# chansoopark98/Deep-Visual-SLAM

Measured on AMD Instinct MI355X. Metric: VO training-step frames/sec (3-frame 640x480 snippets), higher is better.
Workload: dtype f32; 1 GPU; configs[2]/[3]: full 4-scale photometric+smoothness loss, batch 12 per GPU, ResNet-18; per_gpu_batch=12, global_batch=12, num_scales=4, image=640x480, parallelism=dp1, streams=depth | pose | 2x weight-gradient, optimizer=fused Adam pass at lr 0: every step computes from the seeded weights, gpu_max_hw_queues=4

## Files before the change

### deep-visual-slam_amd/csrc/conv_common.h

```cpp
#pragma once
#include "common.h"

namespace dvsconv {

using f32x4 = __attribute__((ext_vector_type(4))) float;
using f32x16 = __attribute__((ext_vector_type(16))) float;

constexpr int BK = 32;
constexpr int LDK = BK + 4;
constexpr int NT = 256;

enum Act { ACT_NONE = 0, ACT_RELU = 1, ACT_ELU = 2, ACT_SIGMOID = 3, ACT_GELU = 4 };
enum Pad { PAD_ZERO = 0, PAD_REFLECT = 1 };
enum InMode {
    IN_NHWC = 0,
    IN_UPCAT = 1,
    IN_PLANAR = 2,
    IN_DGRAD = 3
};

struct ConvShape {
    int B, H, W, Cin;
    int Ho, Wo, Cout;
    int kh, kw, stride, pad;
// ... 161 lines not shown
    return v;
}

__device__ __forceinline__ f32x4 load_dy4(const float* __restrict__ dy, const ConvShape& s, const InXform& t, int b,
                                          int ty, int tx, int co) {
    size_t o = (((size_t)b * s.H + ty) * s.W + tx) * s.Cin + co;
    f32x4 v = *reinterpret_cast<const f32x4*>(dy + o);
    if (t.dact) {
        f32x4 y = *reinterpret_cast<const f32x4*>(t.aux + o);
#pragma unroll
        for (int j = 0; j < 4; ++j) v[j] *= act_grad_from_out(y[j], t.dact);
    }
    return v;
}

__device__ __forceinline__ f32x4 gather_dgrad_raw(const float* __restrict__ dy, const ConvShape& s, const InXform& t,
                                                  int b, int yp, int xp, int ky, int kx, int co, bool& ok, f32x4& yv,
                                                  f32x4& extra) {
    int ty = yp - ky, tx = xp - kx;
    if (s.stride == 2) {
        ok = ok && ((ty | tx) & 1) == 0;
        ty >>= 1;
        tx >>= 1;
    }
    const bool in_y = (unsigned)ty < (unsigned)s.H, in_x = (unsigned)tx < (unsigned)s.W;
    const bool row_ok = ok;
    ok = ok && in_y && in_x;
    size_t o = (((size_t)b * s.H + clampi(ty, s.H)) * s.W + clampi(tx, s.W)) * s.Cin + co;
    f32x4 v = *reinterpret_cast<const f32x4*>(dy + o);
    if (t.dact) yv = *reinterpret_cast<const f32x4*>(t.aux + o);
    extra = f32x4{0.f, 0.f, 0.f, 0.f};
    if (s.pad_mode == PAD_REFLECT) {
        int y = yp - 1, x = xp - 1;
        int ey = (y == 1 && ky == 0) ? 0 : ((y == s.H - 2 && ky == s.kh - 1) ? s.H - 1 : -1);
        int ex = (x == 1 && kx == 0) ? 0 : ((x == s.W - 2 && kx == s.kw - 1) ? s.W - 1 : -1);
        if (row_ok && (ey >= 0 || ex >= 0)) {
            if (ey >= 0 && in_x) extra += load_dy4(dy, s, t, b, ey, tx, co);
            if (ex >= 0 && in_y) extra += load_dy4(dy, s, t, b, ty, ex, co);
            if (ey >= 0 && ex >= 0) extra += load_dy4(dy, s, t, b, ey, ex, co);
        }
    }
    return v;
}

__device__ __forceinline__ f32x4 finalize_dgrad(f32x4 v, const f32x4& yv, const f32x4& extra, bool ok, int dact) {
#pragma unroll
    for (int j = 0; j < 4; ++j) {
        float u = dact ? v[j] * act_grad_from_out(yv[j], dact) : v[j];
        v[j] = (ok ? u : 0.f) + extra[j];
    }
    return v;
}

__device__ __forceinline__ f32x4 gather_planar_raw(const float* __restrict__ x, const ConvShape& s, int b, int iy0,
                                                   int ix0, int k, bool ok, unsigned& mask4, int& ci_out) {
    int kx = k & 7, row = k >> 3;
    int ci = row / s.kh, ky = row - ci * s.kh;
    ci = min(ci, s.Cin - 1);
    ci_out = ci;
    int iy = iy0 + ky;
    bool oky = ok && (unsigned)iy < (unsigned)s.H;
    const float* rowp = x + (((size_t)b * s.Cin + ci) * s.H + clampi(iy, s.H)) * s.W;
    f32x4 v;
    mask4 = 0;
#pragma unroll
    for (int e = 0; e < 4; ++e) {
        int ix = ix0 + kx + e;
        v[e] = rowp[clampi(ix, s.W)];
        mask4 |= (oky && (unsigned)ix < (unsigned)s.W && kx + e < s.kw) ? (1u << e) : 0u;
    }
    return v;
}

template <bool FOLD>
__device__ __forceinline__ f32x4 finalize_planar(f32x4 v, unsigned mask4, float sc, float sh) {
#pragma unroll
    for (int e = 0; e < 4; ++e) {
        float u = FOLD ? v[e] * sc + sh : v[e];
        v[e] = ((mask4 >> e) & 1u) ? u : 0.f;
    }
    return v;
}

template <int TM, int TN>
__device__ __forceinline__ void mfma_stage(const float* __restrict__ As, const float* __restrict__ Bs, int a_row0,
                                           int b_row0, int lane, f32x16 (&acc)[TM][TN]) {
    const int r = lane & 31, h = lane >> 5;
#pragma unroll
    for (int j = 0; j < BK / 8; ++j) {
        f32x4 a[TM], b[TN];
#pragma unroll
        for (int m = 0; m < TM; ++m)
            a[m] = *reinterpret_cast<const f32x4*>(As + (a_row0 + m * 32 + r) * LDK + j * 8 + h * 4);
#pragma unroll
        for (int n = 0; n < TN; ++n)
            b[n] = *reinterpret_cast<const f32x4*>(Bs + (b_row0 + n * 32 + r) * LDK + j * 8 + h * 4);
#pragma unroll
        for (int t = 0; t < 4; ++t)
#pragma unroll
            for (int m = 0; m < TM; ++m)
#pragma unroll
                for (int n = 0; n < TN; ++n)
                    acc[m][n] = __builtin_amdgcn_mfma_f32_32x32x2f32(a[m][t], b[n][t], acc[m][n], 0, 0, 0);
    }
}

using bf16x8 = __attribute__((ext_vector_type(8))) __bf16;
using bf16x4 = __attribute__((ext_vector_type(4))) __bf16;
constexpr int LDKH = BK + 8;
__device__ __forceinline__ bf16x4 to_bf16(f32x4 v) {
    return bf16x4{(__bf16)v[0], (__bf16)v[1], (__bf16)v[2], (__bf16)v[3]};
}
template <int TM, int TN>
__device__ __forceinline__ void mfma_stage_bf16(const __bf16* __restrict__ As, const __bf16* __restrict__ Bs, int a_row0, int b_row0,
                                                int lane, f32x16 (&acc)[TM][TN]) {
    const int r = lane & 31, h = lane >> 5;
#pragma unroll
    for (int j = 0; j < BK / 16; ++j) {
        bf16x8 a[TM], b[TN];
#pragma unroll
        for (int m = 0; m < TM; ++m) a[m] = *reinterpret_cast<const bf16x8*>(As + (a_row0 + m * 32 + r) * LDKH + j * 16 + h * 8);
#pragma unroll
        for (int n = 0; n < TN; ++n) b[n] = *reinterpret_cast<const bf16x8*>(Bs + (b_row0 + n * 32 + r) * LDKH + j * 16 + h * 8);
#pragma unroll
        for (int m = 0; m < TM; ++m)
#pragma unroll
            for (int n = 0; n < TN; ++n) acc[m][n] = __builtin_amdgcn_mfma_f32_32x32x16_bf16(a[m], b[n], acc[m][n], 0, 0, 0);
    }
}

constexpr int OOB_OFF = 0x7ffffff0;
__device__ __forceinline__ __amdgpu_buffer_rsrc_t dma_rsrc(const float* base, size_t bytes) {
    return __builtin_amdgcn_make_buffer_rsrc(const_cast<float*>(base), 0, (int)bytes, 0x00020000);
}
__device__ __forceinline__ void dma16_buf(__amdgpu_buffer_rsrc_t r, int voff_bytes, int soff_bytes, float* lds_wave_base) {
    __builtin_amdgcn_raw_ptr_buffer_load_lds(r, (__attribute__((address_space(3))) void*)lds_wave_base, 16, voff_bytes,
                                             soff_bytes, 0, 0);
}

bool stem_shape(const ConvShape& s);
void stem_wgrad(const float* x, const float* dy, float* dw, const ConvShape& s, const float* sc, const float* sh,
                hipStream_t st);
void stem_fwd(const float* x, const float* w, float* y, float* stats, int stat_groups, const ConvShape& s,
              const float* sc, const float* sh, hipStream_t st);

bool thin_wgrad_shape(const ConvShape& s, const InXform& t);
bool thin_wgrad(const float* x, const float* dy, float* dw, float* dbias, const ConvShape& s, const InXform& t,
                hipStream_t st);
bool thin_fwd(const float* x, const float* w, const float* bias, float* y, const ConvShape& s, const InXform& t, int act,
              hipStream_t st);
bool thin_dgrad(const float* dy, const float* wt, float* dx, const float* y_out, int dact, int B, int H, int W, int Cin,
                int Cout, int split_c1, float* dx_skip, hipStream_t st);

}
```

### deep-visual-slam_amd/csrc/conv_fwd.hip

```cpp
#include "conv_common.h"

#include <cstdlib>
#include <type_traits>

namespace {
using namespace dvsconv;

struct FwdParams {
    const float* x;
    const float* w;
    const float* bias;
    float* y;
    float* stats;
    int stat_split;
    float* y2;
    int split_c1;
    int dbg_nobarrier;
    const float* zero_page;
    const float* res;
    int stat_mask, stat_stride;
    int work_m;
    int ksplit;
    Grid3 g;
    ConvShape s;
// ... 578 lines not shown
    if (W == 3 && x == 1) v += at(y + 1, W + 1) + ((ey >= 0) ? at(ey, W + 1) : f32x4{0.f, 0.f, 0.f, 0.f});
    if (H == 3 && W == 3 && y == 1 && x == 1) v += at(H + 1, W + 1);
    return v;
}
__global__ __launch_bounds__(256) void reflect_fold_kernel(const float* __restrict__ G, float* __restrict__ dx,
                                                           float* __restrict__ dx_skip, int B, int H, int W, int C, int C1) {
    const int cv = C / 4;
    const size_t i = (size_t)blockIdx.x * 256 + threadIdx.x;
    if (C1 == 0) {
        if (i >= (size_t)B * H * W * cv) return;
        const int c = (int)(i % cv) * 4;
        size_t m = i / cv;
        const int x = (int)(m % W);
        m /= W;
        const int y = (int)(m % H), b = (int)(m / H);
        *reinterpret_cast<f32x4*>(dx + (((size_t)b * H + y) * W + x) * C + c) = folded_at(G, b, y, x, c, H, W, C);
        return;
    }
    const int H2 = H >> 1, W2 = W >> 1;
    if (i >= (size_t)B * H2 * W2 * cv) return;
    const int c = (int)(i % cv) * 4;
    size_t m = i / cv;
    const int x2 = (int)(m % W2);
    m /= W2;
    const int y2 = (int)(m % H2), b = (int)(m / H2);
    f32x4 v[4];
#pragma unroll
    for (int q = 0; q < 4; ++q) v[q] = folded_at(G, b, 2 * y2 + (q >> 1), 2 * x2 + (q & 1), c, H, W, C);
    if (c < C1) {
        *reinterpret_cast<f32x4*>(dx + (((size_t)b * H2 + y2) * W2 + x2) * C1 + c) = (v[0] + v[1]) + (v[2] + v[3]);
    } else {
        const int cs = C - C1;
#pragma unroll
        for (int q = 0; q < 4; ++q)
            *reinterpret_cast<f32x4*>(dx_skip + (((size_t)b * H + 2 * y2 + (q >> 1)) * W + 2 * x2 + (q & 1)) * cs + (c - C1)) = v[q];
    }
}

struct PackEntry {
    const float* w;
    float* wt;
    int Cout, Cin, T, wg_begin;
};
__global__ __launch_bounds__(256) void pack_wt_batch_kernel(const PackEntry* __restrict__ tab, int n) {
    __shared__ float tile[32][33];
    __shared__ int s_e;
    if (threadIdx.x == 0) {
        int e = 0;
        while (e + 1 < n && (int)blockIdx.x >= tab[e + 1].wg_begin) ++e;
        s_e = e;
    }
    __syncthreads();
    const PackEntry en = tab[s_e];
    const int tci = (en.Cin + 31) / 32, tco = (en.Cout + 31) / 32;
    int local = blockIdx.x - en.wg_begin;
    const int tap = local / (tci * tco);
    local -= tap * tci * tco;
    const int co0 = (local / tci) * 32, ci0 = (local % tci) * 32;
    const int tx = threadIdx.x & 31, ty = threadIdx.x >> 5;
#pragma unroll
    for (int j = 0; j < 4; ++j) {
        int co = co0 + ty + 8 * j, ci = ci0 + tx;
        tile[ty + 8 * j][tx] = (co < en.Cout && ci < en.Cin) ? en.w[((size_t)co * en.T + tap) * en.Cin + ci] : 0.f;
    }
    __syncthreads();
#pragma unroll
    for (int j = 0; j < 4; ++j) {
        int ci = ci0 + ty + 8 * j, co = co0 + tx;
        if (ci < en.Cin && co < en.Cout) en.wt[((size_t)ci * en.T + tap) * en.Cout + co] = tile[tx][ty + 8 * j];
    }
}

}

extern "C" {

int dvs_reflect_fold(const float* g_padded, float* dx, float* dx_skip, int B, int H, int W, int C, int C1, void* stream) {
    DVS_REQUIRE(g_padded && dx && B > 0 && H >= 3 && W >= 3 && C > 0 && (C & 3) == 0, "dvs_reflect_fold: bad argument");
    DVS_REQUIRE(C1 == 0 || ((C1 & 3) == 0 && C1 <= C && !((H | W) & 1) && (C1 == C || dx_skip)), "dvs_reflect_fold: bad split");
    const size_t n = (C1 == 0 ? (size_t)B * H * W : (size_t)B * (H / 2) * (W / 2)) * (C / 4);
    hipStream_t st = static_cast<hipStream_t>(stream);
    dvs::ProfScope prof(dvs::SLOT_CONV_DGRAD, st);
    hipLaunchKernelGGL(reflect_fold_kernel, dim3((unsigned)((n + 255) / 256)), dim3(256), 0, st, g_padded, dx, dx_skip, B, H, W, C, C1);
    return dvs::check_launch("dvs_reflect_fold");
}

int dvs_act_bwd(const float* dy, const float* y, float* dz, size_t n, int act, float* dbias, int C, void* stream) {
    DVS_REQUIRE(dy && y && dz && n > 0 && (n & 3) == 0 && act >= 0 && act <= 3, "dvs_act_bwd: bad argument");
    DVS_REQUIRE(!dbias || (C >= 4 && (C & 3) == 0 && C / 4 <= 256 && 256 % (C / 4) == 0 && n % C == 0),
                "dvs_act_bwd: the bias gradient needs C/4 to divide 256 (C=%d)", C);
    const size_t nvec = n / 4;
    size_t blocks = (nvec + 255) / 256;
    if (blocks > 512) blocks = 512;
    if (dbias) {
        size_t few = nvec / (256 * 32);
        few = few < 32 ? 32 : few;
        if (blocks > few) blocks = few;
    }
    hipStream_t st = static_cast<hipStream_t>(stream);
    dvs::ProfScope prof(dvs::SLOT_CONV_DGRAD, st);
    hipLaunchKernelGGL(act_bwd_kernel, dim3((unsigned)blocks), dim3(256), 0, st, dy, y, dz, nvec, act, dbias, C);
    return dvs::check_launch("dvs_act_bwd");
}

int dvs_conv2d_pack_wt_batch(const void* table, int n_entries, int total_workgroups, void* stream) {
    DVS_REQUIRE(table && n_entries > 0 && total_workgroups > 0, "dvs_conv2d_pack_wt_batch: bad argument");
    hipLaunchKernelGGL(pack_wt_batch_kernel, dim3(total_workgroups), dim3(256), 0, static_cast<hipStream_t>(stream),
                       static_cast<const PackEntry*>(table), n_entries);
    return dvs::check_launch("dvs_conv2d_pack_wt_batch");
}

int dvs_conv2d_pack_wt(const float* w, float* wt, int Cout, int Cin, int kh, int kw, void* stream) {
    DVS_REQUIRE(w && wt && Cout > 0 && Cin > 0 && kh > 0 && kw > 0, "dvs_conv2d_pack_wt: bad argument");
    dim3 grid((Cin + 31) / 32, (Cout + 31) / 32, kh * kw);
    hipLaunchKernelGGL(pack_wt_kernel, grid, dim3(256), 0, static_cast<hipStream_t>(stream), w, wt, Cout, Cin, kh * kw);
    return dvs::check_launch("dvs_conv2d_pack_wt");
}

int dvs_conv2d_dgrad(const float* dy, const float* wt, float* dx, const dvs_conv_desc* d, const float* y_out,
                     int dact, float* dx_skip, int C1, const float* residual, void* stream) {
    DVS_REQUIRE(dy && wt && dx && d, "dvs_conv2d_dgrad: null pointer");
    DVS_REQUIRE(!residual || (C1 == 0 && residual != dx), "dvs_conv2d_dgrad: a residual excludes the upsample+concat split and may not alias dx");
    DVS_REQUIRE(C1 == 0 || (d->stride == 1 && (d->H & 1) == 0 && (d->W & 1) == 0 && C1 <= d->Cin &&
                            (C1 == d->Cin || dx_skip != nullptr)),
                "dvs_conv2d_dgrad: bad upsample+concat split");
    DVS_REQUIRE(d->stride == 1 || d->stride == 2, "dvs_conv2d_dgrad: stride %d (1 or 2 supported)", d->stride);
    DVS_REQUIRE((d->Cout & 3) == 0 && (d->Cin & 3) == 0, "dvs_conv2d_dgrad: channel counts must be multiples of 4");
    DVS_REQUIRE(d->pad_mode == PAD_ZERO || (d->pad_mode == 2 && d->pad == 0 && d->stride == 1 && d->H > 2 && d->W > 2 && !dact && !C1) ||
                    (d->pad_mode == PAD_REFLECT && d->pad == 1 && d->kh == 3 && d->kw == 3 && d->stride == 1 && d->H >= 2 && d->W >= 2),
                "dvs_conv2d_dgrad: reflect mode is ReflectionPad2d(1) + 3x3 stride 1 only; pad_mode 2 = pre-padded input, pad 0");
    DVS_REQUIRE(!dact || y_out, "dvs_conv2d_dgrad: activation gradient needs the forward output");
    DVS_REQUIRE((double)d->B * d->H * d->W * (d->Cin > d->Cout ? d->Cin : d->Cout) < 2147483648.0,
                "dvs_conv2d_dgrad: tensors must have fewer than 2^31 elements (32-bit gather offsets)");
    FwdParams p{};
    p.x = dy; p.w = wt; p.y = dx;
    p.stat_split = 0x7fffffff;
    ConvShape& s = p.s;
    int Ho = (d->H + 2 * d->pad - d->kh) / d->stride + 1, Wo = (d->W + 2 * d->pad - d->kw) / d->stride + 1;
    s.B = d->B;
    s.Ho = d->H; s.Wo = d->W; s.Cout = d->Cin;
    s.H = Ho; s.W = Wo; s.Cin = d->Cout;
    s.kh = d->kh; s.kw = d->kw; s.stride = d->stride; s.pad = d->pad; s.pad_mode = d->pad_mode;
    if (d->pad_mode == 2) {
        s.pad_mode = PAD_ZERO;
        p.work_m = d->B * (d->H - 2) * (d->W - 2);
    }
    s.Ktot = d->kh * d->kw * d->Cout;
    p.t.aux = y_out;
    p.t.dact = dact;
    p.y2 = dx_skip;
    p.split_c1 = C1;
    p.res = residual;
    hipStream_t st = static_cast<hipStream_t>(stream);
    if (!residual && d->pad_mode == PAD_REFLECT && d->kh == 3 && d->kw == 3 && d->stride == 1 && d->pad == 1 &&
        thin_dgrad(dy, wt, dx, y_out, dact, d->B, d->H, d->W, d->Cin, d->Cout, C1, dx_skip, st))
        return dvs::check_launch("dvs_conv2d_dgrad");
    launch_mode<IN_DGRAD, false>(p, st, dvs::SLOT_CONV_DGRAD);
    return dvs::check_launch("dvs_conv2d_dgrad");
}

int dvs_conv2d_fwd(const float* x, const float* w, const float* bias, float* y, const dvs_conv_desc* d,
                   const dvs_conv_fusion* f, void* stream) {
    DVS_REQUIRE(x && w && y && d, "dvs_conv2d_fwd: null pointer");
    DVS_REQUIRE(d->B > 0 && d->H > 0 && d->W > 0 && d->Cin > 0 && d->Cout > 0 && d->kh > 0 && d->kw > 0 &&
                    d->stride > 0 && d->pad >= 0,
                "dvs_conv2d_fwd: bad descriptor");
    FwdParams p{};
    p.x = x; p.w = w; p.bias = bias; p.y = y;
    p.stat_split = 0x7fffffff;
    ConvShape& s = p.s;
    s.B = d->B; s.H = d->H; s.W = d->W; s.Cin = d->Cin; s.Cout = d->Cout;
    s.kh = d->kh; s.kw = d->kw; s.stride = d->stride; s.pad = d->pad; s.pad_mode = d->pad_mode;
    s.Ho = (d->H + 2 * d->pad - d->kh) / d->stride + 1;
    s.Wo = (d->W + 2 * d->pad - d->kw) / d->stride + 1;
    DVS_REQUIRE(s.Ho > 0 && s.Wo > 0, "dvs_conv2d_fwd: empty output");
    DVS_REQUIRE((double)d->B * d->H * d->W * d->Cin < 2147483648.0 && (double)d->B * s.Ho * s.Wo * d->Cout < 2147483648.0,
                "dvs_conv2d_fwd: tensors must have fewer than 2^31 elements (32-bit gather offsets)");
    DVS_REQUIRE(d->pad_mode == PAD_ZERO || (d->pad < d->H && d->pad < d->W), "dvs_conv2d_fwd: reflect pad too large");
    int planar = 0;
    if (f) {
        p.t.x2 = f->x2; p.t.C1 = f->C1; p.t.in_scale = f->in_scale; p.t.in_shift = f->in_shift;
        p.t.in_relu = f->in_relu; planar = f->nchw_planar;
        p.act = f->act; p.stats = f->stats; p.res = f->residual;
        DVS_REQUIRE(f->act >= 0 && f->act <= ACT_GELU, "dvs_conv2d_fwd: unknown activation %d", f->act);
        DVS_REQUIRE(!(f->residual && f->stats), "dvs_conv2d_fwd: residual and stats are exclusive (inference vs training)");
        DVS_REQUIRE(f->stat_groups >= 0 && f->stat_groups <= 2 && (f->stat_groups != 2 || (d->B % 2) == 0),
                    "dvs_conv2d_fwd: stat_groups is 0, 1 or 2 (2 needs an even batch)");
        p.stat_split = (f->stat_groups == 2) ? (d->B / 2) * s.Ho * s.Wo : 0x7fffffff;
        if (f->stats && f->stat_slots > 1) {
            DVS_REQUIRE(f->stat_slots <= 64 && (f->stat_slots & (f->stat_slots - 1)) == 0 && !f->nchw_planar,
                        "dvs_conv2d_fwd: stat_slots must be a power of two <= 64 (NHWC input only)");
            p.stat_mask = f->stat_slots - 1;
            p.stat_stride = (f->stat_groups == 2 ? 2 : 1) * 2 * d->Cout;
        }
        DVS_REQUIRE(!(f->x2) || (f->C1 > 0 && (d->H & 1) == 0 && (d->W & 1) == 0 &&
                                 ((f->C1 == d->Cin && (f->C1 & 3) == 0) || (f->C1 < d->Cin && (f->C1 % BK) == 0))),
                    "dvs_conv2d_fwd: upsample+concat needs C1 %% 32 == 0 (or C1 == Cin) and even H, W");
        DVS_REQUIRE(!(f->x2 && planar), "dvs_conv2d_fwd: planar input cannot be concatenated");
        DVS_REQUIRE((f->in_scale == nullptr) == (f->in_shift == nullptr), "dvs_conv2d_fwd: in_scale/in_shift come together");
    }
    if (planar) {
        DVS_REQUIRE(d->kw <= 8 && d->pad_mode == PAD_ZERO, "dvs_conv2d_fwd: planar input supports kw <= 8, zero padding");
        s.Ktot = d->Cin * d->kh * 8;
    } else {
        DVS_REQUIRE((d->Cin & 3) == 0, "dvs_conv2d_fwd: NHWC input needs Cin %% 4 == 0 (got %d)", d->Cin);
        s.Ktot = d->kh * d->kw * d->Cin;
    }
    hipStream_t st = static_cast<hipStream_t>(stream);
    const bool fold = p.t.in_scale != nullptr;
    static const bool stem16 = [] { const char* e = getenv("DVS_BF16_STEM"); return e && e[0] == '1'; }();
    if (planar && stem_shape(s) && !p.t.in_relu && bias == nullptr && p.act == ACT_NONE && !p.res && !(stem16 && dvs::precision_bf16())) {
        dvs::ProfScope prof(dvs::SLOT_CONV_FWD, st);
        prof.work(2.0 * s.B * s.Ho * s.Wo * s.Cout * (double)s.Cin * s.kh * s.kw);
        stem_fwd(x, w, y, p.stats, f && f->stat_groups == 2 ? 2 : 1, s, p.t.in_scale, p.t.in_shift, st);
    } else if (!planar && !p.stats && !p.res && thin_fwd(x, w, bias, y, s, p.t, p.act, st)) {
    } else if (planar) {
        if (fold) launch_mode<IN_PLANAR, true>(p, st, dvs::SLOT_CONV_FWD);
        else launch_mode<IN_PLANAR, false>(p, st, dvs::SLOT_CONV_FWD);
    } else if (p.t.x2) {
        if (fold) launch_mode<IN_UPCAT, true>(p, st, dvs::SLOT_CONV_FWD);
        else launch_mode<IN_UPCAT, false>(p, st, dvs::SLOT_CONV_FWD);
    } else {
        if (fold) launch_mode<IN_NHWC, true>(p, st, dvs::SLOT_CONV_FWD);
        else launch_mode<IN_NHWC, false>(p, st, dvs::SLOT_CONV_FWD);
    }
    return dvs::check_launch("dvs_conv2d_fwd");
}

}
```

### deep-visual-slam_amd/csrc/conv_wgrad.hip

```cpp
#include "conv_common.h"

#include <cstdlib>

namespace {
using namespace dvsconv;

constexpr int BP = 32;

struct WgradParams {
    const float* x;
    const float* dy;
    float* dw;
    float* dbias;
    ConvShape s;
    InXform t;
    int m_per_split;
    Grid3 g;
    int dbg;
    float* part;
    size_t part_bytes;
};

template <int TM, int TN, int WN>
__device__ __forceinline__ void wgrad_store(const WgradParams& p, const f32x16 (&acc)[TM][TN], int tile, int bid_z, int co0, int k0, int wave,
// ... 521 lines not shown
    f32x16 acc[TM][TN];
#pragma unroll
    for (int m = 0; m < TM; ++m)
#pragma unroll
        for (int n = 0; n < TN; ++n)
#pragma unroll
            for (int i = 0; i < 16; ++i) acc[m][n][i] = 0.f;

    const int r = lane & 31, h = lane >> 5;
    const int a_col = wm * TM * 32 + r, b_col = wn * TN * 32 + r;
    fill_ring(0, m_begin);
    fill_ring(1, m_begin + PTG);
    __syncthreads();
    if (m_begin < m_end) issue_stage(m_begin, 0);
    asm volatile("s_waitcnt vmcnt(0)" ::: "memory");
    __syncthreads();
    int buf = 0, stage = 0;
#pragma unroll 1
    for (int mb = m_begin; mb < m_end; mb += BPD, ++stage) {
        if ((stage & (SPR - 1)) == 0 && stage > 0) fill_ring(((stage / SPR) + 1) & 1, m_begin + ((stage / SPR) + 1) * PTG);
        if (mb + BPD < m_end) issue_stage(mb + BPD, buf ^ 1);
#pragma unroll
        for (int t = 0; t < BPD / 2; ++t) {
            float a[TM], b[TN];
#pragma unroll
            for (int m = 0; m < TM; ++m) a[m] = Ds[buf][2 * t + h][a_col + m * 32];
#pragma unroll
            for (int n = 0; n < TN; ++n) b[n] = Xs[buf][2 * t + h][b_col + n * 32];
#pragma unroll
            for (int m = 0; m < TM; ++m)
#pragma unroll
                for (int n = 0; n < TN; ++n)
                    acc[m][n] = __builtin_amdgcn_mfma_f32_32x32x2f32(a[m], b[n], acc[m][n], 0, 0, 0);
        }
        asm volatile("s_waitcnt vmcnt(0)" ::: "memory");
        __syncthreads();
        buf ^= 1;
    }
    wgrad_store<TM, TN, WN>(p, acc, bid_y * p.g.x + bid_x, bid_z, co0, k0, wave, lane);
}

template <int BM, int BN, int WM, int WN, int MODE, bool FOLD>
void launch_cfg(WgradParams p, hipStream_t st, size_t* need = nullptr) {
    const int M = p.s.B * p.s.Ho * p.s.Wo;
    const int tiles = ((p.s.Cout + BM - 1) / BM) * ((p.s.Ktot + BN - 1) / BN);
    static const int wg_target = [] { const char* e = getenv("DVS_WGRAD_WGS"); return e ? atoi(e) : 1024; }();
    int splits = (wg_target + tiles - 1) / tiles;
    splits = max(1, min(splits, (M + 255) / 256));
    int mps = ((M + splits - 1) / splits + BP - 1) / BP * BP;
    splits = (M + mps - 1) / mps;
    p.m_per_split = mps;
    dim3 grid((p.s.Cout + BM - 1) / BM, (p.s.Ktot + BN - 1) / BN, splits);
    static const int xcd_on = [] { const char* e = getenv("DVS_CONV_XCD"); return !(e && e[0] == '0') ? 1 : 0; }();
    p.g = Grid3{(int)grid.x, (int)grid.y, (int)grid.z, xcd_on};
    const size_t slab = (size_t)grid.x * grid.y * grid.z * BM * BN * sizeof(float);
    if (need) {
        *need = slab;
        return;
    }
    if (p.part && p.part_bytes < slab) p.part = nullptr;
    struct Reduce {
        const WgradParams& p; dim3 g; hipStream_t st;
        ~Reduce() {
            if (p.part)
                hipLaunchKernelGGL((wgrad_reduce_kernel<BM, BN, WM, WN>), dim3(g.x * g.y * (BM * BN / NT)), dim3(NT), 0, st, p.part, p.dw,
                                   p.s.Cout, p.s.Ktot, (int)g.x, (int)(g.x * g.y), (int)g.z);
        }
    } reduce_after{p, grid, st};
    dvs::ProfScope prof(dvs::SLOT_CONV_WGRAD, st);
    const double k_real = (MODE == IN_PLANAR) ? (double)p.s.Cin * p.s.kh * p.s.kw : (double)p.s.Ktot;
    prof.work(2.0 * M * p.s.Cout * k_real);
    if constexpr (MODE == IN_PLANAR) {
        if (dvs::precision_bf16()) {
            hipLaunchKernelGGL((conv_wgrad_kernel<BM, BN, WM, WN, MODE, FOLD, true>), dim3(grid.x * grid.y * grid.z), dim3(NT), 0, st, p);
            return;
        }
    }
    if constexpr (!FOLD && MODE != IN_PLANAR) {
        if (dvs::precision_bf16()) {
            hipLaunchKernelGGL((conv_wgrad_kernel<BM, BN, WM, WN, MODE, FOLD, true>), dim3(grid.x * grid.y * grid.z), dim3(NT), 0, st, p);
            return;
        }
        static const bool dma = [] { const char* e = getenv("DVS_CONV_DMA"); return !(e && e[0] == '0'); }();
        static const int dbg = dvs::experiment_flags("DVS_CONV_DEBUG_NOBARRIER");
        p.dbg = dbg & 4;
        if (dma && MODE == IN_NHWC && p.s.pad_mode == PAD_ZERO && p.t.dact == 0 && p.dbias == nullptr && p.s.kh * p.s.kw <= 30 &&
            (double)p.s.B * p.s.H * p.s.W * p.s.Cin < 536870912.0 && (double)M * p.s.Cout < 536870912.0) {
            static const int bpd = [] { const char* e = getenv("DVS_WGRAD_BP"); return e ? atoi(e) : 16; }();
            if constexpr (BM >= 64) {
                if (bpd == 16) {
                    hipLaunchKernelGGL((conv_wgrad_dma_kernel<BM, BN, WM, WN, IN_NHWC, 16>), dim3(grid.x * grid.y * grid.z), dim3(NT), 0, st, p);
                    return;
                }
            }
            hipLaunchKernelGGL((conv_wgrad_dma_kernel<BM, BN, WM, WN, IN_NHWC, 32>), dim3(grid.x * grid.y * grid.z), dim3(NT), 0, st, p);
            return;
        }
    }
    if constexpr (!FOLD && MODE != IN_PLANAR && BM >= 64) {
        static const bool gen = [] { const char* e = getenv("DVS_WGRAD_GEN"); return !(e && e[0] == '0'); }();
        static const bool dma2 = [] { const char* e = getenv("DVS_CONV_DMA"); return !(e && e[0] == '0'); }();
        if (gen && dma2 && (MODE == IN_UPCAT || p.s.pad_mode == PAD_REFLECT) && p.t.dact == 0 && p.dbias == nullptr &&
            p.s.kh == 3 && p.s.kw == 3 && p.s.stride == 1 && (double)M * p.s.Cout < 536870912.0) {
            hipLaunchKernelGGL((conv_wgrad_dma_gen_kernel<BM, BN, WM, WN, MODE>), dim3(grid.x * grid.y * grid.z), dim3(NT), 0, st, p);
            return;
        }
    }
    hipLaunchKernelGGL((conv_wgrad_kernel<BM, BN, WM, WN, MODE, FOLD>), dim3(grid.x * grid.y * grid.z), dim3(NT), 0, st, p);
}

template <int MODE, bool FOLD>
void launch_mode(const WgradParams& p, hipStream_t st, size_t* need = nullptr) {
    if (p.s.Cout > 64) launch_cfg<128, 128, 2, 2, MODE, FOLD>(p, st, need);
    else if (p.s.Cout > 32) launch_cfg<64, 128, 1, 4, MODE, FOLD>(p, st, need);
    else launch_cfg<32, 128, 1, 4, MODE, FOLD>(p, st, need);
}

}

extern "C" {

static int wgrad_impl(const float* x, const float* dy, float* dw, float* dbias, const dvs_conv_desc* d, const dvs_conv_fusion* f,
                      const float* y_out, int dact, float* workspace, size_t workspace_bytes, size_t* need, void* stream) {
    DVS_REQUIRE(need || (x && dy && dw), "dvs_conv2d_wgrad: null pointer");
    DVS_REQUIRE(d, "dvs_conv2d_wgrad: null descriptor");
    DVS_REQUIRE((d->Cout & 3) == 0, "dvs_conv2d_wgrad: Cout must be a multiple of 4 (got %d)", d->Cout);
    DVS_REQUIRE(!dact || y_out, "dvs_conv2d_wgrad: activation gradient needs the forward output");
    WgradParams p{};
    p.x = x; p.dy = dy; p.dw = dw; p.dbias = dbias;
    p.part = workspace; p.part_bytes = workspace_bytes;
    ConvShape& s = p.s;
    s.B = d->B; s.H = d->H; s.W = d->W; s.Cin = d->Cin; s.Cout = d->Cout;
    s.kh = d->kh; s.kw = d->kw; s.stride = d->stride; s.pad = d->pad; s.pad_mode = d->pad_mode;
    s.Ho = (d->H + 2 * d->pad - d->kh) / d->stride + 1;
    s.Wo = (d->W + 2 * d->pad - d->kw) / d->stride + 1;
    int planar = 0;
    if (f) {
        p.t.x2 = f->x2; p.t.C1 = f->C1; p.t.in_scale = f->in_scale; p.t.in_shift = f->in_shift;
        p.t.in_relu = f->in_relu; planar = f->nchw_planar;
    }
    p.t.aux = y_out;
    p.t.dact = dact;
    if (planar) {
        DVS_REQUIRE(d->kw <= 8 && d->pad_mode == PAD_ZERO, "dvs_conv2d_wgrad: planar input supports kw <= 8, zero padding");
        s.Ktot = d->Cin * d->kh * 8;
    } else {
        DVS_REQUIRE((d->Cin & 3) == 0, "dvs_conv2d_wgrad: NHWC input needs Cin %% 4 == 0 (got %d)", d->Cin);
        s.Ktot = d->kh * d->kw * d->Cin;
    }
    hipStream_t st = static_cast<hipStream_t>(stream);
    const bool fold = p.t.in_scale != nullptr;
    if (need) *need = 0;
    static const bool stem16 = [] { const char* e = getenv("DVS_BF16_STEM"); return e && e[0] == '1'; }();
    if (planar && stem_shape(s) && dact == 0 && dbias == nullptr && !p.t.in_relu && !(stem16 && dvs::precision_bf16())) {
        if (need) return DVS_OK;
        dvs::ProfScope prof(dvs::SLOT_CONV_WGRAD, st);
        prof.work(2.0 * s.B * s.Ho * s.Wo * s.Cout * (double)s.Cin * s.kh * s.kw);
        stem_wgrad(x, dy, dw, s, p.t.in_scale, p.t.in_shift, st);
    } else if (!planar && thin_wgrad_shape(s, p.t)) {
        if (need) return DVS_OK;
        thin_wgrad(x, dy, dw, dbias, s, p.t, st);
    } else if (planar) {
        if (fold) launch_mode<IN_PLANAR, true>(p, st, need);
        else launch_mode<IN_PLANAR, false>(p, st, need);
    } else if (p.t.x2) {
        if (fold) launch_mode<IN_UPCAT, true>(p, st, need);
        else launch_mode<IN_UPCAT, false>(p, st, need);
    } else {
        if (fold) launch_mode<IN_NHWC, true>(p, st, need);
        else launch_mode<IN_NHWC, false>(p, st, need);
    }
    return need ? DVS_OK : dvs::check_launch("dvs_conv2d_wgrad");
}

size_t dvs_conv2d_wgrad_workspace(const dvs_conv_desc* d, const dvs_conv_fusion* f, int dact, int with_bias) {
    size_t need = 0;
    static float dummy;
    if (wgrad_impl(nullptr, nullptr, nullptr, with_bias ? &dummy : nullptr, d, f, dact ? &dummy : nullptr, dact, nullptr, 0, &need, nullptr) != DVS_OK)
        return 0;
    return need;
}

int dvs_conv2d_wgrad(const float* x, const float* dy, float* dw, float* dbias, const dvs_conv_desc* d, const dvs_conv_fusion* f,
                     const float* y_out, int dact, float* workspace, size_t workspace_bytes, void* stream) {
    if (workspace) {
        const size_t need = dvs_conv2d_wgrad_workspace(d, f, dact, dbias != nullptr);
        DVS_REQUIRE(workspace_bytes >= need, "dvs_conv2d_wgrad: workspace of %zu bytes, %zu needed", workspace_bytes, need);
    }
    return wgrad_impl(x, dy, dw, dbias, d, f, y_out, dact, workspace, workspace_bytes, nullptr, stream);
}

}
```

Measured before the change: 1531 frames/s.

## Add dedicated pointwise (1x1) conv GEMM kernels for fwd, dgrad and wgrad

Adds specialised MFMA GEMM kernels for 1x1 convolutions (ResNet downsample shortcuts and 512-channel stride-1 1x1 layers). They use buffer-load-to-LDS DMA pipelining and swizzled LDS, and fuse BN statistics, bias/activation, stride-2 scatter with residual add, and split-K wgrad with atomics. The aim is to avoid the generic im2col-style implicit GEMM overhead on these layers. The cost is extra code paths that depend on atomic accumulation and only activate for specific channel counts.

After: 1540 frames/s, median of 6. About the same (+0.6%).

```diff
diff --git a/deep-visual-slam_amd/csrc/conv_common.h b/deep-visual-slam_amd/csrc/conv_common.h
--- a/deep-visual-slam_amd/csrc/conv_common.h
+++ b/deep-visual-slam_amd/csrc/conv_common.h
@@ -337,4 +337,10 @@
 bool thin_dgrad(const float* dy, const float* wt, float* dx, const float* y_out, int dact, int B, int H, int W, int Cin,
                 int Cout, int split_c1, float* dx_skip, hipStream_t st);
 
-}
+bool pw_shape(const ConvShape& s);
+void pw_fwd(const float* x, const float* w, const float* bias, float* y, float* stats, int stat_split, int stat_mask,
+            int stat_stride, const ConvShape& s, int act, hipStream_t st);
+void pw_dgrad(const float* dz, const float* wt, float* dx, const float* residual, const ConvShape& s, hipStream_t st);
+void pw_wgrad(const float* x, const float* dz, float* dw, float* dbias, const ConvShape& s, hipStream_t st);
+
+}
diff --git a/deep-visual-slam_amd/csrc/conv_fwd.hip b/deep-visual-slam_amd/csrc/conv_fwd.hip
--- a/deep-visual-slam_amd/csrc/conv_fwd.hip
+++ b/deep-visual-slam_amd/csrc/conv_fwd.hip
@@ -754,6 +754,15 @@
     p.split_c1 = C1;
     p.res = residual;
     hipStream_t st = static_cast<hipStream_t>(stream);
+    if (!dact && C1 == 0 && d->kh == 1 && d->kw == 1) {
+        ConvShape c{};
+        c.B = d->B; c.H = d->H; c.W = d->W; c.Cin = d->Cin; c.Ho = Ho; c.Wo = Wo; c.Cout = d->Cout;
+        c.kh = 1; c.kw = 1; c.stride = d->stride; c.pad = d->pad; c.pad_mode = d->pad_mode; c.Ktot = d->Cin;
+        if (pw_shape(c)) {
+            pw_dgrad(dy, wt, dx, residual, c, st);
+            return dvs::check_launch("dvs_conv2d_dgrad");
+        }
+    }
     if (!residual && d->pad_mode == PAD_REFLECT && d->kh == 3 && d->kw == 3 && d->stride == 1 && d->pad == 1 &&
         thin_dgrad(dy, wt, dx, y_out, dact, d->B, d->H, d->W, d->Cin, d->Cout, C1, dx_skip, st))
         return dvs::check_launch("dvs_conv2d_dgrad");
@@ -811,7 +820,9 @@
     hipStream_t st = static_cast<hipStream_t>(stream);
     const bool fold = p.t.in_scale != nullptr;
     static const bool stem16 = [] { const char* e = getenv("DVS_BF16_STEM"); return e && e[0] == '1'; }();
-    if (planar && stem_shape(s) && !p.t.in_relu && bias == nullptr && p.act == ACT_NONE && !p.res && !(stem16 && dvs::precision_bf16())) {
+    if (!planar && !p.t.x2 && !fold && !p.res && (p.stats || s.stride == 1) && pw_shape(s)) {
+        pw_fwd(x, w, bias, y, p.stats, p.stat_split, p.stat_mask, p.stat_stride, s, p.act, st);
+    } else if (planar && stem_shape(s) && !p.t.in_relu && bias == nullptr && p.act == ACT_NONE && !p.res && !(stem16 && dvs::precision_bf16())) {
         dvs::ProfScope prof(dvs::SLOT_CONV_FWD, st);
         prof.work(2.0 * s.B * s.Ho * s.Wo * s.Cout * (double)s.Cin * s.kh * s.kw);
         stem_fwd(x, w, y, p.stats, f && f->stat_groups == 2 ? 2 : 1, s, p.t.in_scale, p.t.in_shift, st);
diff --git a/deep-visual-slam_amd/csrc/conv_pw.hip b/deep-visual-slam_amd/csrc/conv_pw.hip
--- /dev/null
+++ b/deep-visual-slam_amd/csrc/conv_pw.hip
@@ -0,0 +1,392 @@
+#include "conv_common.h"
+
+#include <cstdlib>
+
+namespace {
+using namespace dvsconv;
+
+constexpr int PW_BM = 64, PW_BN = 64;
+constexpr int PW_STAGE = (PW_BM + PW_BN) * BK;
+constexpr int PW_DEPTH = 2;
+constexpr int PW_INS = 4;
+constexpr int PW_LDC = PW_BN + 4;
+constexpr int PW_WG_PIX = 1024;
+
+__device__ __forceinline__ void pw_wait_barrier(int later) {
+    if (later <= 0) asm volatile("s_waitcnt vmcnt(0) lgkmcnt(0)\n\ts_barrier" ::: "memory");
+    else if (later == 1) asm volatile("s_waitcnt vmcnt(4) lgkmcnt(0)\n\ts_barrier" ::: "memory");
+    else if (later == 2) asm volatile("s_waitcnt vmcnt(8) lgkmcnt(0)\n\ts_barrier" ::: "memory");
+    else asm volatile("s_waitcnt vmcnt(12) lgkmcnt(0)\n\ts_barrier" ::: "memory");
+    static_assert(PW_INS == 4, "the vmcnt immediates above count 4 loads per stage");
+}
+
+struct PwGemmParams {
+    const float* a;
+    const float* b;
+    const float* bias;
+    const float* res;
+    float* y;
+    float* stats;
+    int stat_split, stat_mask, stat_stride, act;
+    int M, N, K;
+    int Hs, Ws;
+    int H, W, stride;
+    int a_pixels;
+    int gy, remap;
+};
+
+template <int D>
+__device__ __forceinline__ void pw_gemm_tile(const __amdgpu_buffer_rsrc_t ra, const __amdgpu_buffer_rsrc_t rb, const int (&a_off)[2],
+                                             const int (&b_off)[2], int nst, float* smem, int wave, int lane, int wm, int wn,
+                                             f32x16& acc) {
+    auto issue = [&](int st) {
+        float* As = smem + (st % D) * PW_STAGE;
+        float* Bs = As + PW_BM * BK;
+        const int soff = st * BK * 4;
+#pragma unroll
+        for (int j = 0; j < 2; ++j) dma16_buf(ra, a_off[j], soff, As + (wave * 2 + j) * 8 * BK);
+#pragma unroll
+        for (int j = 0; j < 2; ++j) dma16_buf(rb, b_off[j], soff, Bs + (wave * 2 + j) * 8 * BK);
+    };
+    const int pre = min(nst, D);
+    for (int st = 0; st < pre; ++st) issue(st);
+    const int r = lane & 31, h = lane >> 5;
+    const int arow = wm * 32 + r, brow = wn * 32 + r;
+    const int asw = (arow >> 1) & 7, bsw = (brow >> 1) & 7;
+#pragma unroll 1
+    for (int i = 0; i < nst; ++i) {
+        pw_wait_barrier(i == 0 ? pre - 1 : min(nst - 1 - i, D - 2));
+        if (i >= 1 && i - 1 + D < nst) issue(i - 1 + D);
+        const float* As = smem + (i % D) * PW_STAGE;
+        const float* Bs = As + PW_BM * BK;
+#pragma unroll
+        for (int j = 0; j < BK / 8; ++j) {
+            const f32x4 a = *reinterpret_cast<const f32x4*>(As + arow * BK + (((2 * j + h) ^ asw) << 2));
+            const f32x4 b = *reinterpret_cast<const f32x4*>(Bs + brow * BK + (((2 * j + h) ^ bsw) << 2));
+#pragma unroll
+            for (int t = 0; t < 4; ++t) acc = __builtin_amdgcn_mfma_f32_32x32x2f32(a[t], b[t], acc, 0, 0, 0);
+        }
+    }
+}
+
+template <bool DGRAD>
+__global__ __launch_bounds__(NT) void conv_pw_kernel(PwGemmParams p) {
+    constexpr int D = PW_DEPTH;
+    extern __shared__ __attribute__((aligned(16))) float smem[];
+    const int tid = threadIdx.x, lane = tid & 63;
+    const int wave = __builtin_amdgcn_readfirstlane(tid >> 6);
+    const int wm = wave >> 1, wn = wave & 1;
+    const int gx = (p.M + PW_BM - 1) / PW_BM;
+    const int lg = xcd_logical(blockIdx.x, gx * p.gy, p.remap);
+    const int bid_y = lg % p.gy, bid_x = lg / p.gy;
+    const int m0 = bid_x * PW_BM, n0 = bid_y * PW_BN;
+
+    const int rsub = lane >> 3, slot = lane & 7;
+    int a_off[2], b_off[2];
+#pragma unroll
+    for (int j = 0; j < 2; ++j) {
+        const int row = (wave * 2 + j) * 8 + rsub;
+        const int q = (slot ^ ((row >> 1) & 7)) << 4;
+        const int m = m0 + row;
+        int pix = min(m, p.M - 1);
+        if (!DGRAD && p.stride == 2) {
+            const int b = pix / (p.Hs * p.Ws), rem = pix - b * (p.Hs * p.Ws);
+            const int oy = rem / p.Ws, ox = rem - oy * p.Ws;
+            pix = (b * p.H + 2 * oy) * p.W + 2 * ox;
+        }
+        a_off[j] = m < p.M ? pix * p.K * 4 + q : OOB_OFF;
+        const int n = n0 + row;
+        b_off[j] = n < p.N ? n * p.K * 4 + q : OOB_OFF;
+    }
+    const __amdgpu_buffer_rsrc_t ra = dma_rsrc(p.a, (size_t)p.a_pixels * p.K * 4);
+    const __amdgpu_buffer_rsrc_t rb = dma_rsrc(p.b, (size_t)p.N * p.K * 4);
+
+    f32x16 acc;
+#pragma unroll
+    for (int i = 0; i < 16; ++i) acc[i] = 0.f;
+    pw_gemm_tile<D>(ra, rb, a_off, b_off, p.K / BK, smem, wave, lane, wm, wn, acc);
+
+    const int ln = lane & 31, lh = lane >> 5;
+    if constexpr (!DGRAD) {
+        const int n = n0 + wn * 32 + ln;
+        const bool n_ok = n < p.N;
+        const int mb = m0 + wm * 32;
+        const float bv = (p.bias && n_ok) ? p.bias[n] : 0.f;
+        const bool plain = p.bias == nullptr && p.act == ACT_NONE;
+#pragma unroll
+        for (int i = 0; i < 16; ++i) {
+            const int m = mb + 4 * lh + (i & 3) + 8 * (i >> 2);
+            if (m < p.M && n_ok) p.y[(size_t)m * p.N + n] = plain ? acc[i] : apply_act(acc[i] + bv, p.act);
+        }
+        if (p.stats) {
+            const bool lo = mb >= p.stat_split, hi = mb + 31 >= p.stat_split;
+            float s0 = 0.f, q0 = 0.f, s1 = 0.f, q1 = 0.f;
+            if (lo == hi) {
+#pragma unroll
+                for (int i = 0; i < 16; ++i) {
+                    s0 += acc[i];
+                    q0 += acc[i] * acc[i];
+                }
+                if (lo) {
+                    s1 = s0;
+                    q1 = q0;
+                }
+            } else {
+#pragma unroll
+                for (int i = 0; i < 16; ++i) {
+                    const bool second = mb + 4 * lh + (i & 3) + 8 * (i >> 2) >= p.stat_split;
+                    const float v = acc[i];
+                    s0 += second ? 0.f : v;
+                    q0 += second ? 0.f : v * v;
+                    s1 += second ? v : 0.f;
+                    q1 += second ? v * v : 0.f;
+                }
+            }
+            float* st = p.stats + (size_t)(bid_x & p.stat_mask) * p.stat_stride;
+            if (!lo) {
+                s0 += __shfl_xor(s0, 32, 64);
+                q0 += __shfl_xor(q0, 32, 64);
+                if (lh == 0 && n_ok) {
+                    atomicAdd(st + n, s0);
+                    atomicAdd(st + p.N + n, q0);
+                }
+            }
+            if (hi) {
+                s1 += __shfl_xor(s1, 32, 64);
+                q1 += __shfl_xor(q1, 32, 64);
+                if (lh == 0 && n_ok) {
+                    atomicAdd(st + 2 * p.N + n, s1);
+                    atomicAdd(st + 3 * p.N + n, q1);
+                }
+            }
+        }
+    } else {
+        float* Cs = smem;
+        int* rowpix = reinterpret_cast<int*>(smem + PW_BM * PW_LDC);
+        int* rowfl = rowpix + PW_BM;
+        __syncthreads();
+#pragma unroll
+        for (int i = 0; i < 16; ++i)
+            Cs[(wm * 32 + 4 * lh + (i & 3) + 8 * (i >> 2)) * PW_LDC + wn * 32 + ln] = acc[i];
+        if (tid < PW_BM) {
+            const int m = m0 + tid;
+            int pix = m, fl = 0;
+            if (p.stride == 2 && m < p.M) {
+                const int b = m / (p.Hs * p.Ws), rem = m - b * (p.Hs * p.Ws);
+                const int oy = rem / p.Ws, ox = rem - oy * p.Ws;
+                pix = (b * p.H + 2 * oy) * p.W + 2 * ox;
+                fl = (2 * ox + 1 < p.W ? 1 : 0) | (2 * oy + 1 < p.H ? 2 : 0);
+            }
+            rowpix[tid] = m < p.M ? pix * p.N : -1;
+            rowfl[tid] = fl;
+        }
+        __syncthreads();
+        const int c = (tid & 15) * 4;
+        const f32x4 zero = {0.f, 0.f, 0.f, 0.f};
+        if (n0 + c < p.N) {
+#pragma unroll
+            for (int ps = 0; ps < PW_BM / 16; ++ps) {
+                const int row = ps * 16 + (tid >> 4);
+                const int base = rowpix[row], fl = rowfl[row];
+                if (base < 0) continue;
+                const int o00 = base + n0 + c, o01 = o00 + p.N, o10 = o00 + p.W * p.N, o11 = o10 + p.N;
+                f32x4 v = *reinterpret_cast<const f32x4*>(Cs + row * PW_LDC + c);
+                f32x4 r01 = zero, r10 = zero, r11 = zero;
+                if (p.res) {
+                    v += *reinterpret_cast<const f32x4*>(p.res + o00);
+                    if (fl & 1) r01 = *reinterpret_cast<const f32x4*>(p.res + o01);
+                    if (fl & 2) r10 = *reinterpret_cast<const f32x4*>(p.res + o10);
+                    if (fl == 3) r11 = *reinterpret_cast<const f32x4*>(p.res + o11);
+                }
+                *reinterpret_cast<f32x4*>(p.y + o00) = v;
+                if (fl & 1) *reinterpret_cast<f32x4*>(p.y + o01) = r01;
+                if (fl & 2) *reinterpret_cast<f32x4*>(p.y + o10) = r10;
+                if (fl == 3) *reinterpret_cast<f32x4*>(p.y + o11) = r11;
+            }
+        }
+    }
+}
+
+struct PwWgradParams {
+    const float* x;
+    const float* dz;
+    float* dw;
+    float* dbias;
+    int M, Cout, Cin;
+    int Hs, Ws, H, W, stride, x_pixels;
+    int tiles_ci, tiles, m_per_split, remap;
+};
+
+__global__ __launch_bounds__(NT) void conv_pw_wgrad_kernel(PwWgradParams p) {
+    constexpr int D = 3, PB = 32;
+    static_assert(PB * (PW_BM + PW_BN) == PW_STAGE, "a stage is 32 pixels of both operands");
+    extern __shared__ __attribute__((aligned(16))) float smem[];
+    int* tab = reinterpret_cast<int*>(smem + D * PW_STAGE);
+    const int tid = threadIdx.x, lane = tid & 63;
+    const int wave = __builtin_amdgcn_readfirstlane(tid >> 6);
+    const int wm = wave >> 1, wn = wave & 1;
+    const int lg = xcd_logical(blockIdx.x, gridDim.x, p.remap);
+    const int tile = lg % p.tiles, split = lg / p.tiles;
+    const int co0 = (tile / p.tiles_ci) * PW_BM, ci0 = (tile % p.tiles_ci) * PW_BN;
+    const int m_begin = split * p.m_per_split, m_end = min(p.M, m_begin + p.m_per_split);
+    const int nst = (m_end - m_begin + PB - 1) / PB;
+
+    for (int i = tid; i < nst * PB; i += NT) {
+        const int m = m_begin + i;
+        int pix = m;
+        if (p.stride == 2 && m < m_end) {
+            const int b = m / (p.Hs * p.Ws), rem = m - b * (p.Hs * p.Ws);
+            const int oy = rem / p.Ws, ox = rem - oy * p.Ws;
+            pix = (b * p.H + 2 * oy) * p.W + 2 * ox;
+        }
+        tab[i] = m < m_end ? pix * p.Cin * 4 : OOB_OFF;
+    }
+    __syncthreads();
+
+    const __amdgpu_buffer_rsrc_t rd = dma_rsrc(p.dz, (size_t)p.M * p.Cout * 4);
+    const __amdgpu_buffer_rsrc_t rx = dma_rsrc(p.x, (size_t)p.x_pixels * p.Cin * 4);
+    const int prow = lane >> 4, chunk = lane & 15;
+    const bool co_ok = co0 + chunk * 4 < p.Cout;
+    const int x_col = (ci0 + chunk * 4) * 4;
+    auto issue = [&](int st) {
+        float* Ds = smem + (st % D) * PW_STAGE;
+        float* Xs = Ds + PB * PW_BM;
+#pragma unroll
+        for (int j = 0; j < 2; ++j) {
+            const int i = st * PB + (wave * 2 + j) * 4 + prow;
+            const int m = m_begin + i;
+            const int d_off = (m < m_end && co_ok) ? (m * p.Cout + co0 + chunk * 4) * 4 : OOB_OFF;
+            dma16_buf(rd, d_off, 0, Ds + (wave * 2 + j) * 4 * PW_BM);
+        }
+#pragma unroll
+        for (int j = 0; j < 2; ++j) {
+            const int e = tab[st * PB + (wave * 2 + j) * 4 + prow];
+            dma16_buf(rx, e == OOB_OFF ? OOB_OFF : e + x_col, 0, Xs + (wave * 2 + j) * 4 * PW_BN);
+        }
+    };
+    const int pre = min(nst, D);
+    for (int st = 0; st < pre; ++st) issue(st);
+
+    f32x16 acc;
+#pragma unroll
+    for (int i = 0; i < 16; ++i) acc[i] = 0.f;
+    const int r = lane & 31, h = lane >> 5;
+    const bool want_bias = p.dbias != nullptr && ci0 == 0;
+    float bsum = 0.f;
+#pragma unroll 1
+    for (int i = 0; i < nst; ++i) {
+        pw_wait_barrier(i == 0 ? pre - 1 : min(nst - 1 - i, D - 2));
+        if (i >= 1 && i - 1 + D < nst) issue(i - 1 + D);
+        const float* Ds = smem + (i % D) * PW_STAGE;
+        const float* Xs = Ds + PB * PW_BM;
+#pragma unroll
+        for (int t = 0; t < PB / 2; ++t) {
+            const float a = Ds[(2 * t + h) * PW_BM + wm * 32 + r];
+            const float b = Xs[(2 * t + h) * PW_BN + wn * 32 + r];
+            acc = __builtin_amdgcn_mfma_f32_32x32x2f32(a, b, acc, 0, 0, 0);
+        }
+        if (want_bias) {
+#pragma unroll
+            for (int t = 0; t < PB / 4; ++t) bsum += Ds[(wave * (PB / 4) + t) * PW_BM + lane];
+        }
+    }
+    __syncthreads();
+    float* Cs = smem;
+    float* red = smem + PW_BM * PW_BN;
+    const int ln = lane & 31, lh = lane >> 5;
+#pragma unroll
+    for (int i = 0; i < 16; ++i) Cs[(wm * 32 + 4 * lh + (i & 3) + 8 * (i >> 2)) * PW_BN + wn * 32 + ln] = acc[i];
+    if (want_bias) red[wave * 64 + lane] = bsum;
+    __syncthreads();
+    const int rot = (split * 7) & (PW_BM - 1);
+#pragma unroll 4
+    for (int ps = 0; ps < PW_BM / 4; ++ps) {
+        const int row = (ps * 4 + wave + rot) & (PW_BM - 1);
+        if (co0 + row < p.Cout) atomicAdd(p.dw + (size_t)(co0 + row) * p.Cin + ci0 + lane, Cs[row * PW_BN + lane]);
+    }
+    if (want_bias && tid < PW_BM && co0 + tid < p.Cout)
+        atomicAdd(p.dbias + co0 + tid, ((red[tid] + red[64 + tid]) + red[128 + tid]) + red[192 + tid]);
+}
+
+bool pw_enabled() {
+    static const bool on = [] { const char* e = getenv("DVS_CONV_PW"); return !(e && e[0] == '0'); }();
+    return on;
+}
+int pw_xcd_remap() {
+    static const int on = [] { const char* e = getenv("DVS_CONV_XCD"); return !(e && e[0] == '0') ? 1 : 0; }();
+    return on;
+}
+
+void pw_launch_gemm(bool dgrad, PwGemmParams& p, hipStream_t st) {
+    const int gx = (p.M + PW_BM - 1) / PW_BM;
+    p.gy = (p.N + PW_BN - 1) / PW_BN;
+    p.remap = pw_xcd_remap();
+    const int nst = p.K / BK;
+    size_t lds = (size_t)(nst < PW_DEPTH ? nst : PW_DEPTH) * PW_STAGE * sizeof(float);
+    const size_t epi = (size_t)(PW_BM * PW_LDC + 2 * PW_BM) * sizeof(float);
+    if (dgrad && lds < epi) lds = epi;
+    if (dgrad) hipLaunchKernelGGL(conv_pw_kernel<true>, dim3(gx * p.gy), dim3(NT), lds, st, p);
+    else hipLaunchKernelGGL(conv_pw_kernel<false>, dim3(gx * p.gy), dim3(NT), lds, st, p);
+}
+
+}
+
+namespace dvsconv {
+
+bool pw_shape(const ConvShape& s) {
+    if (!pw_enabled() || dvs::precision_bf16() || dvs::deterministic()) return false;
+    if (s.kh != 1 || s.kw != 1 || s.pad != 0 || s.pad_mode != PAD_ZERO || (s.stride != 1 && s.stride != 2)) return false;
+    if (s.Cin != 64 && s.Cin != 128 && s.Cin != 256 && s.Cin != 512) return false;
+    if (s.Cout <= 0 || (s.Cout % 32) != 0) return false;
+    if (s.stride == 1 && s.Cin != 512) return false;
+    const double lim = 2147483648.0 / 4;
+    return (double)s.B * s.H * s.W * s.Cin < lim && (double)s.B * s.Ho * s.Wo * s.Cout < lim && (double)s.Cout * s.Cin < lim;
+}
+
+void pw_fwd(const float* x, const float* w, const float* bias, float* y, float* stats, int stat_split, int stat_mask,
+            int stat_stride, const ConvShape& s, int act, hipStream_t st) {
+    PwGemmParams p{};
+    p.a = x; p.b = w; p.bias = bias; p.y = y; p.stats = stats;
+    p.stat_split = stat_split; p.stat_mask = stat_mask; p.stat_stride = stat_stride; p.act = act;
+    p.M = s.B * s.Ho * s.Wo; p.N = s.Cout; p.K = s.Cin;
+    p.Hs = s.Ho; p.Ws = s.Wo; p.H = s.H; p.W = s.W; p.stride = s.stride;
+    p.a_pixels = s.B * s.H * s.W;
+    dvs::ProfScope prof(dvs::SLOT_CONV_FWD, st);
+    prof.work(2.0 * p.M * s.Cout * (double)s.Cin);
+    pw_launch_gemm(false, p, st);
+}
+
+void pw_dgrad(const float* dz, const float* wt, float* dx, const float* residual, const ConvShape& s, hipStream_t st) {
+    PwGemmParams p{};
+    p.a = dz; p.b = wt; p.res = residual; p.y = dx;
+    p.stat_split = 0x7fffffff;
+    p.M = s.B * s.Ho * s.Wo; p.N = s.Cin; p.K = s.Cout;
+    p.Hs = s.Ho; p.Ws = s.Wo; p.H = s.H; p.W = s.W; p.stride = s.stride;
+    p.a_pixels = p.M;
+    dvs::ProfScope prof(dvs::SLOT_CONV_DGRAD, st);
+    prof.work(2.0 * s.B * s.H * s.W * s.Cin * (double)s.Cout / (s.stride * s.stride));
+    pw_launch_gemm(true, p, st);
+}
+
+void pw_wgrad(const float* x, const float* dz, float* dw, float* dbias, const ConvShape& s, hipStream_t st) {
+    PwWgradParams p{};
+    p.x = x; p.dz = dz; p.dw = dw; p.dbias = dbias;
+    p.M = s.B * s.Ho * s.Wo; p.Cout = s.Cout; p.Cin = s.Cin;
+    p.Hs = s.Ho; p.Ws = s.Wo; p.H = s.H; p.W = s.W; p.stride = s.stride;
+    p.x_pixels = s.B * s.H * s.W;
+    p.tiles_ci = s.Cin / PW_BN;
+    p.tiles = ((s.Cout + PW_BM - 1) / PW_BM) * p.tiles_ci;
+    int splits = (512 + p.tiles - 1) / p.tiles;
+    splits = max(1, min(splits, (p.M + 31) / 32));
+    int mps = ((p.M + splits - 1) / splits + 31) / 32 * 32;
+    mps = min(mps, PW_WG_PIX);
+    splits = (p.M + mps - 1) / mps;
+    p.m_per_split = mps;
+    p.remap = pw_xcd_remap();
+    dvs::ProfScope prof(dvs::SLOT_CONV_WGRAD, st);
+    prof.work(2.0 * p.M * s.Cout * (double)s.Cin);
+    const size_t lds = (size_t)3 * PW_STAGE * sizeof(float) + PW_WG_PIX * sizeof(int);
+    hipLaunchKernelGGL(conv_pw_wgrad_kernel, dim3(p.tiles * splits), dim3(NT), lds, st, p);
+}
+
+}
diff --git a/deep-visual-slam_amd/csrc/conv_wgrad.hip b/deep-visual-slam_amd/csrc/conv_wgrad.hip
--- a/deep-visual-slam_amd/csrc/conv_wgrad.hip
+++ b/deep-visual-slam_amd/csrc/conv_wgrad.hip
@@ -697,7 +697,9 @@
     const bool fold = p.t.in_scale != nullptr;
     if (need) *need = 0;
     static const bool stem16 = [] { const char* e = getenv("DVS_BF16_STEM"); return e && e[0] == '1'; }();
-    if (planar && stem_shape(s) && dact == 0 && dbias == nullptr && !p.t.in_relu && !(stem16 && dvs::precision_bf16())) {
+    if (!need && !workspace && !planar && !p.t.x2 && !fold && dact == 0 && pw_shape(s)) {
+        pw_wgrad(x, dy, dw, dbias, s, st);
+    } else if (planar && stem_shape(s) && dact == 0 && dbias == nullptr && !p.t.in_relu && !(stem16 && dvs::precision_bf16())) {
         if (need) return DVS_OK;
         dvs::ProfScope prof(dvs::SLOT_CONV_WGRAD, st);
         prof.work(2.0 * s.B * s.Ho * s.Wo * s.Cout * (double)s.Cin * s.kh * s.kw);
```
